# risingwavelabs/risingwave

Measured on NVIDIA H100. Metric: Nexmark q7/q8-shaped streaming HashJoin input rows/s, higher is better.
Workload: dtype int64

## Files before the change

risingwave_b200/csrc/join.cu:

```cuda
#include <algorithm>
#include <chrono>
#include <cstdio>
#include <cstdlib>
#include <memory>
#include <mutex>
#include <thread>

#include <cub/device/device_radix_sort.cuh>
#include <cub/device/device_scan.cuh>

#include "common.cuh"

namespace rw {

#define J_EMPTY 0x8000000000000000ull
#define J_NIL 0x7fffffffu
#define J_DEAD 0x80000000u
#define J_MAX_OUT (2 * RW_MAX_COLS)
#define J_HDR 16
#define W_EMPTY 0x7fffffffull
#define W_COUNT_ONE (1ull << 33)
#define W_IL_LIVE (1ull << 31)
#define W_IL_DEAD (2ull << 31)
#define W_IL_MASK (3ull << 31)
// ... 1268 lines not shown
      DevBuf b;
      const cudaError_t e = b.reserve((size_t)U_SEG_RECS * 48);
      std::lock_guard<std::mutex> g(mu);
      if (e == cudaSuccess) { spare = std::move(b); spare_ready = true; } else { cudaGetLastError(); }
      worker_running = false;
    });
  }
  int ensure(uint64_t rows, cudaStream_t st) {
    if (!table.p) {
      RW_CUDA(table.reserve(U_MAX_SEGS * sizeof(void*)));
      RW_CUDA(cudaMemsetAsync(table.p, 0, U_MAX_SEGS * sizeof(void*), st));
    }
    while (cap() < rows) {
      if (segs.size() >= U_MAX_SEGS) return fail(RW_ERR_OOM, "join side exceeds 2^31 log rows");
      DevBuf sg;
      if (worker.joinable()) worker.join();
      {
        std::lock_guard<std::mutex> g(mu);
        if (spare_ready) { sg = std::move(spare); spare_ready = false; prefetched++; }
      }
      if (!sg.p) {
        cudaError_t e = sg.reserve((size_t)U_SEG_RECS * 48);
        if (e != cudaSuccess) { cudaGetLastError(); return fail(RW_ERR_OOM, std::string("join log segment: ") + cudaGetErrorString(e)); }
        stalls++;
      }
      void* ptr = sg.p;
      RW_CUDA(cudaMemcpyAsync(table.as<uint8_t>() + segs.size() * sizeof(void*), &ptr, sizeof(void*), cudaMemcpyHostToDevice, st));
      segs.push_back(std::move(sg));
    }
    return RW_OK;
  }
};

struct JoinSideHost {
  int n_cols = 0;
  std::vector<int> types;
  SegLog log;
  GrowBuf recs;
  DevBuf slots;
  DevBuf pools;
  int stride = 0, bstride = 0;
  uint64_t row_cap = 0;
  uint64_t n_rows = 0;
  uint64_t slot_cap = 0;
  uint64_t keys_upper = 0;
};

struct JoinPending {
  int S = 0, set = 0, grid = 0;
  DevChunk ch;
  cudaStream_t st = nullptr;
  int64_t out_base = 0;
  bool plain = true, counted = false, sync_done = false;
  uint32_t pool_chunk = 0;
  uint64_t seq_base = 0, ids_before = 0, keys_before = 0;
  unsigned long long tag = 0;
  int64_t rows = 0;
  unsigned long long nullm = 0;
};

struct rwgpu_join {
  JoinPlanDev plan;
  DevBuf plan_dev, status;
  PinnedBuf status_host;
  JoinSideHost side[2];
  cudaStream_t stream = nullptr, s_h2d = nullptr, s_d2h = nullptr;
  cudaEvent_t ev_h2d[8] = {nullptr}, ev_main[8] = {nullptr};
  std::vector<int> out_types;
  int chunk_size = 1024;
  bool fast_inner = false;
  bool w8_ok[2] = {false, false};
  W8Plan w8[2];
  bool uni = false;
  int uni_is = 1;
  DevBuf uni_buckets, uni_counters;
  uint64_t uni_cap = 0, uni_keys = 0, uni_keys_exact = 0;
  uint64_t uni_dead[2] = {0, 0};
  uint64_t compactions = 0;
  DevBuf uni_wk_entry, uni_wk_mask;
  int64_t uni_wk_cap = 0;
  JoinPending pending[2];
  int n_pending = 0;
  cudaEvent_t pend_ev[2] = {nullptr, nullptr};
  cudaStream_t last_st = nullptr;
  cudaEvent_t order_ev = nullptr;
  bool wm_pending[2] = {false, false};
  int wm_key_pos[2] = {0, 0};
  int64_t wm_value[2] = {0, 0};
  uint64_t wm_cleanings = 0;
  uint64_t launches = 0;
  uint64_t seq = 0;
  unsigned long long status_tag = 0;
  unsigned long long call_null_mask = 0;
  bool out_rows_cumulative = false;
  KernelProf prof;
  DevBuf sk, sk_alt, packed, offs, mslot, gtable, cub_tmp;
  int64_t scratch_rows = 0;
  uint64_t gcap = 0;
  size_t cub_bytes = 0;
  struct OutSet {
    DevBuf out_ops, out_vis, out_col[J_MAX_OUT], out_valid[J_MAX_OUT], out_bits[J_MAX_OUT], out_visbits;
    int64_t out_cap = 0;
    unsigned long long valid_dirty = 0;
  } oset[2];
  int cur = 0;
  OutSet& os() { return oset[cur]; }
// ... 283 lines not shown
static int join_order(rwgpu_join* h, cudaStream_t st) {
  if (h->last_st && h->last_st != st) {
    if (!h->order_ev) RW_CUDA(cudaEventCreateWithFlags(&h->order_ev, cudaEventDisableTiming));
    RW_CUDA(cudaEventRecord(h->order_ev, h->last_st));
    RW_CUDA(cudaStreamWaitEvent(st, h->order_ev, 0));
  }
  h->last_st = st;
  return RW_OK;
}

static int uni_tail_grid(int64_t n) {
  static int max_blocks = 0;
  if (!max_blocks) {
    int dev = 0, sms = 0, per_sm = 0;
    cudaGetDevice(&dev);
    cudaDeviceGetAttribute(&sms, cudaDevAttrMultiProcessorCount, dev);
    int a = 0, b = 0;
    cudaOccupancyMaxActiveBlocksPerMultiprocessor(&a, uni_tail_kernel<false>, 256, 0);
    cudaOccupancyMaxActiveBlocksPerMultiprocessor(&b, uni_tail_kernel<true>, 256, 0);
    per_sm = std::max(1, std::min(std::min(a, b), 3));
    max_blocks = std::max(1, sms * per_sm);
  }
  return (int)std::max<int64_t>(1, std::min<int64_t>((n + 255) / 256, max_blocks));
}

static int uni_launch_main(rwgpu_join* h, const JoinPending& pd, bool probe_only, unsigned long long tag) {
  UniDev t = uni_dev(h);
  const JoinPlanDev* pdev = h->plan_dev.as<JoinPlanDev>();
  JoinStatus* ds = h->status.as<JoinStatus>();
  int S = pd.S;
  const bool is_row = S == h->uni_is;
  JoinOutDev od = out_dev(h);
  UniWork wk;
  wk.entry = h->uni_wk_entry.as<UniDefer>();
  wk.mask = h->uni_wk_mask.as<uint8_t>();
  W8Plan w = h->w8[S];
  h->prof.begin(pd.st);
  if (pd.plain) {
    PlainChunk pc;
    pc.ops = pd.ch.ops;
    for (int c = 0; c < 4; c++) pc.c[c] = c < w.n_u ? (const unsigned long long*)pd.ch.cols[c].data : nullptr;
    pc.key = (const unsigned long long*)pd.ch.cols[w.key_col].data;
    pc.n = pd.ch.n;
    pc.n_dev = pd.ch.n_dev;
    UniOwn own;
    own.log = t.log[S];
    own.log_cap = t.log_cap[S];
    own.pools = t.pools[S];
    own.log_next = t.log_next[S];
    PlainOut po;
    po.ops = od.ops;
    po.vis = od.vis;
    for (int c = 0; c < 4; c++) {
      po.ucol[c] = (c < w.n_u && w.u_out[c] >= 0) ? (unsigned long long*)od.col[w.u_out[c]] : nullptr;
      po.mcol[c] = (c < w.n_m && w.m_out[c] >= 0) ? (unsigned long long*)od.col[w.m_out[c]] : nullptr;
    }
    po.capacity = od.capacity;
    auto hot = probe_only ? (is_row ? uni_hot_kernel<true, true> : uni_hot_kernel<true, false>)
                          : (is_row ? uni_hot_kernel<false, true> : uni_hot_kernel<false, false>);
    hot<<<pd.grid, JF_BLOCK, 0, pd.st>>>(pc, t.buckets, t.cap, own, po, wk, ds, pd.seq_base, pd.out_base, pd.pool_chunk);
  } else {
    if (probe_only) uni_slow_kernel<true><<<jgrid(pd.ch.n, 256), 256, 0, pd.st>>>(pdev, w, S, pd.ch, t, od, ds, pd.seq_base, pd.out_base);
    else uni_slow_kernel<false><<<jgrid(pd.ch.n, 256), 256, 0, pd.st>>>(pdev, w, S, pd.ch, t, od, ds, pd.seq_base, pd.out_base);
  }
  h->prof.end(pd.st);
  RW_CUDA(cudaGetLastError());
  DevChunk chv = pd.ch;
  uint64_t seq_base = pd.seq_base;
  int64_t out_base = pd.out_base;
  JoinStatus* slot = (JoinStatus*)(h->status_host.as<uint8_t>() + 512 * pd.set);
  int reset = 3;
  unsigned int* done = (unsigned int*)(h->uni_counters.as<unsigned long long>() + 6);
  const int tg = uni_tail_grid(pd.ch.n);
  if (probe_only) uni_tail_kernel<true><<<tg, 256, 0, pd.st>>>(pdev, w, S, chv, t, od, wk, ds, seq_base, out_base, slot, tag, reset, done);
  else uni_tail_kernel<false><<<tg, 256, 0, pd.st>>>(pdev, w, S, chv, t, od, wk, ds, seq_base, out_base, slot, tag, reset, done);
  RW_CUDA(cudaGetLastError());
  h->launches += 2;
  return RW_OK;
}

static int join_plain_chunk(DevChunk* ch, bool device_count, cudaStream_t st, bool* plain) {
  *plain = ch->vis_bits == nullptr;
  for (int c = 0; c < ch->n_cols && *plain; c++)
    *plain = !ch->cols[c].valid_bits && !ch->cols[c].valid_bytes && (((uintptr_t)ch->cols[c].data & 7) == 0);
  if (!ch->n_dev || (device_count && *plain)) return RW_OK;
  int64_t nh = 0;
  RW_CUDA(cudaMemcpyAsync(&nh, ch->n_dev, sizeof(nh), cudaMemcpyDeviceToHost, st));
  RW_CUDA(cudaStreamSynchronize(st));
  if (nh < 0 || nh > ch->n) return fail(RW_ERR_INVALID, "device row count out of range");
  ch->n = nh;
  ch->n_dev = nullptr;
  return RW_OK;
}

static double uni_now_ms() { return std::chrono::duration<double, std::milli>(std::chrono::steady_clock::now().time_since_epoch()).count(); }
static const bool uni_trace = getenv("RWGPU_TRACE") != nullptr;

static int uni_enqueue(rwgpu_join* h, int S, const DevChunk& ch_in, cudaStream_t st, int64_t out_base, JoinPending* pd) {
  const double tr0 = uni_trace ? uni_now_ms() : 0.0;
  DevChunk ch = ch_in;
  bool plain_cols;
  int rc = join_plain_chunk(&ch, true, st, &plain_cols);
  if (rc != RW_OK) return rc;
  const bool counted = ch.n_dev != nullptr;
  const int64_t n = ch.n;
  JoinSideHost& own = h->side[S];
  const int grid = (int)std::max<int64_t>(1, std::min<int64_t>((n + 63) / 64, U_MAX_GRID));
  uint32_t pool_chunk = 32;
  while (pool_chunk < 256 && (int64_t)pool_chunk * grid * 8 < 4 * n) pool_chunk <<= 1;
  const uint64_t id_slack = (uint64_t)grid * 8 * pool_chunk;
  rc = join_grow_store(h, S, own.n_rows + (uint64_t)n + id_slack);
  if (rc != RW_OK) return rc;
  rc = uni_grow_table(h, h->uni_keys + (uint64_t)n);
  if (rc != RW_OK) return rc;
  rc = join_ensure_out(h, out_base + n + std::max<int64_t>(n / 2, 4096), st, out_base);
  if (rc != RW_OK) return rc;
  if (plain_cols && n > h->uni_wk_cap) {
    RW_CUDA(cudaDeviceSynchronize());
    const int64_t cap = n + n / 4 + 64;
    RW_CUDA(h->uni_wk_entry.reserve((size_t)cap * sizeof(UniDefer)));
    RW_CUDA(h->uni_wk_mask.reserve((size_t)(cap + 7) / 8 + 16));
    h->uni_wk_cap = cap;
  }
  rc = join_order(h, st);
  if (rc != RW_OK) return rc;
  const double tr1 = uni_trace ? uni_now_ms() : 0.0;
  pd->S = S;
  pd->ch = ch;
  pd->st = st;
  pd->out_base = out_base;
  pd->set = h->cur;
  pd->plain = plain_cols;
  pd->counted = counted;
  pd->grid = grid;
  pd->pool_chunk = pool_chunk;
  pd->seq_base = h->seq;
  pd->tag = ++h->status_tag;
  pd->ids_before = own.n_rows;
  pd->keys_before = h->uni_keys;
  h->seq += (uint64_t)n;
  own.n_rows += (uint64_t)n + id_slack;
  h->uni_keys += (uint64_t)n;
  rc = uni_launch_main(h, *pd, false, pd->tag);
  if (rc != RW_OK) return rc;
  if (!h->pend_ev[pd->set]) RW_CUDA(cudaEventCreateWithFlags(&h->pend_ev[pd->set], cudaEventDisableTiming));
  RW_CUDA(cudaEventRecord(h->pend_ev[pd->set], st));
  if (uni_trace)
    fprintf(stderr, "  [uni_enqueue S=%d n=%lld set=%d] grow/ensure %.3f ms, launch %.3f ms (log segs %zu/%zu, cap %llu keys<=%llu)\n", S, (long long)n,
            pd->set, tr1 - tr0, uni_now_ms() - tr1, h->side[0].log.segs.size(), h->side[1].log.segs.size(), (unsigned long long)h->uni_cap,
            (unsigned long long)h->uni_keys);
  return RW_OK;
}

static int uni_finish(rwgpu_join* h, const JoinPending& pd, int64_t* out_rows, unsigned long long* null_mask) {
  cudaStream_t st = pd.st;
  JoinStatus* ds = h->status.as<JoinStatus>();
  JoinStatus* slot = (JoinStatus*)(h->status_host.as<uint8_t>() + 512 * pd.set);
  JoinStatus hs;
  const double tr0 = uni_trace ? uni_now_ms() : 0.0;
  RW_CUDA(cudaEventSynchronize(h->pend_ev[pd.set]));
  const double tr1 = uni_trace ? uni_now_ms() : 0.0;
  int rc;
  if (*(volatile unsigned long long*)(slot + 1) != pd.tag) return fail(RW_ERR_CUDA, "join status block was not published");
  memcpy(&hs, slot, sizeof(JoinStatus));
  unsigned int err = hs.err;
  const unsigned long long first_null = hs.null_mask;
  const bool first_match = hs.pad != 0;
  const unsigned long long first_del = hs.n_del;
  const bool redone = (hs.err & JERR_OUT_CAPACITY) != 0;
  if (redone) {
    const int64_t extras = (int64_t)hs.out_rows, n = pd.ch.n;
    RW_CUDA(cudaMemsetAsync(&ds->err, 0, 4, st));
    rc = join_ensure_out(h, pd.out_base + n + extras + (int64_t)pd.grid * 8 * U_XCHUNK, st, pd.out_base);
    if (rc != RW_OK) return rc;
    const unsigned long long tag2 = ++h->status_tag;
    rc = uni_launch_main(h, pd, true, tag2);
    if (rc != RW_OK) return rc;
    RW_CUDA(cudaStreamSynchronize(st));
    if (*(volatile unsigned long long*)(slot + 1) != tag2) return fail(RW_ERR_CUDA, "join status block was not published");
    memcpy(&hs, slot, sizeof(JoinStatus));
    err = (err & ~JERR_OUT_CAPACITY) | hs.err;
    hs.null_mask |= first_null & ~(1ull << 63);
    hs.pad = hs.pad || first_match;
    hs.n_del = first_del;
  }
  for (int s = 0; s < 2; s++) h->uni_dead[s] = hs.n_dead[s];
  {
    JoinSideHost& own = h->side[pd.S];
    const uint64_t n = (uint64_t)pd.ch.n, slack = (uint64_t)pd.grid * 8 * pd.pool_chunk;
    const uint64_t rows_now = hs.log_next[pd.S] + (own.n_rows - (pd.ids_before + n + slack));
    const uint64_t keys_now = hs.n_keys[0] + (h->uni_keys - (pd.keys_before + n));
    for (int i = 0; i < h->n_pending; i++) {
      h->pending[i].ids_before += rows_now - own.n_rows;
      h->pending[i].keys_before += keys_now - h->uni_keys;
    }
    own.n_rows = rows_now;
    h->uni_keys = keys_now;
    h->uni_keys_exact = hs.n_keys[0];
  }
  hs.err = err;
  rc = join_check_err(h, hs, st);
  if (rc != RW_OK) return rc;
  const int64_t n_eff = pd.counted ? (int64_t)hs.n_in : pd.ch.n;
  *out_rows = (hs.pad != 0 || hs.out_rows) ? n_eff + (int64_t)hs.out_rows : 0;
  h->call_null_mask |= hs.null_mask;
  *null_mask = h->call_null_mask;
  h->os().valid_dirty |= hs.null_mask & ((1ull << 63) - 1);
  if (hs.n_del) h->call_had_deletes = true;
  if (uni_trace)
    fprintf(stderr, "  [uni_finish S=%d set=%d] wait %.3f ms, rest %.3f ms (redo %d, extras %llu, n_del %llu, out %lld)\n", pd.S, pd.set, tr1 - tr0,
            uni_now_ms() - tr1, (int)redone, (unsigned long long)hs.out_rows,
            (unsigned long long)hs.n_del, (long long)*out_rows);
  return RW_OK;
}

static int join_push_dev_uni(rwgpu_join* h, int S, const DevChunk& ch_in, cudaStream_t st, int64_t out_base, int64_t* out_rows,
                             unsigned long long* null_mask) {
  if (h->n_pending) return fail(RW_ERR_INVALID, "collect the outstanding asynchronous pushes first");
  JoinPending pd;
  int rc = uni_enqueue(h, S, ch_in, st, out_base, &pd);
  if (rc != RW_OK) return rc;
  return uni_finish(h, pd, out_rows, null_mask);
}

static int join_push_dev(rwgpu_join* h, int S, const DevChunk& ch_in, cudaStream_t st, int64_t out_base, int64_t* out_rows,
                         unsigned long long* null_mask) {
  *out_rows = 0;
  DevChunk ch = ch_in;
  if (ch.n <= 0) return RW_OK;
  if (ch.n >= (1ll << 31)) return fail(RW_ERR_INVALID, "chunk too large");
  if (h->uni) return join_push_dev_uni(h, S, ch_in, st, out_base, out_rows, null_mask);
  bool plain_cols;
  int rc = join_plain_chunk(&ch, false, st, &plain_cols);
  if (rc != RW_OK) return rc;
  if (ch.n == 0) return RW_OK;
  const int64_t n = ch.n;
  JoinSideHost& own = h->side[S];
  static const bool trace = getenv("RWGPU_TRACE") != nullptr;
  auto now = []() { return std::chrono::duration<double, std::milli>(std::chrono::steady_clock::now().time_since_epoch()).count(); };
  const double tt0 = now();
  const uint64_t cap0 = own.slot_cap, rcap0 = own.row_cap;
  rc = join_grow_store(h, S, own.n_rows + (uint64_t)n);
  if (rc != RW_OK) return rc;
  rc = join_grow_slots(h, S, own.keys_upper + (uint64_t)n);
  if (rc != RW_OK) return rc;
  if (trace)
    fprintf(stderr, "  [push_dev S=%d n=%lld] grow %.3f ms (slot_cap %llu->%llu, row_cap %llu->%llu, n_rows %llu keys %llu)\n", S, (long long)n,
            now() - tt0, (unsigned long long)cap0, (unsigned long long)own.slot_cap, (unsigned long long)rcap0,
            (unsigned long long)own.row_cap, (unsigned long long)own.n_rows, (unsigned long long)own.keys_upper);
  JoinStatus* ds = h->status.as<JoinStatus>();
  const JoinPlanDev* pd = h->plan_dev.as<JoinPlanDev>();
  const uint64_t seq_base = h->seq;
  h->seq += (uint64_t)n;
  JoinStatus hs;
  if (h->fast_inner) {
    const bool use_w8 = h->w8_ok[S] && plain_cols;
    if (use_w8) {
      rc = join_ensure_out(h, out_base + n + std::max<int64_t>(n / 2, 4096), st, out_base);
      if (rc != RW_OK) return rc;
      const int grid = jgrid(n, JF_BLOCK);
      auto launch = [&](bool probe_only, uint32_t store_base) {
        if (probe_only)
          join_inner_w8p_kernel<true><<<grid, JF_BLOCK, 0, st>>>(pd, h->w8[S], S, ch, side_dev(h, S), side_dev(h, 1 - S), out_dev(h), ds,
                                                                  store_base, seq_base, out_base);
        else
          join_inner_w8p_kernel<false><<<grid, JF_BLOCK, 0, st>>>(pd, h->w8[S], S, ch, side_dev(h, S), side_dev(h, 1 - S), out_dev(h), ds,
                                                                   store_base, seq_base, out_base);
      };
      h->prof.begin(st);
      launch(false, (uint32_t)own.n_rows);
      h->prof.end(st);
      const unsigned long long tag = ++h->status_tag;
      join_inner_delete_kernel<<<jgrid(n, 256), 256, 0, st>>>(pd, S, ch, side_dev(h, S), ds, seq_base, h->status_host.as<JoinStatus>(), tag, 3);
      RW_CUDA(cudaGetLastError());
      h->launches += 2;
      rc = join_read_status(h, st, &hs, 3, tag);
      if (rc != RW_OK) return rc;
      const uint64_t stored = hs.n_store, keys = hs.n_keys[S];
      if (hs.n_del) h->call_had_deletes = true;
      unsigned int err = hs.err;
      if (hs.err & JERR_OUT_CAPACITY) {
        const int64_t extras = (int64_t)hs.out_rows;
        RW_CUDA(cudaMemsetAsync(&ds->out_rows, 0, 8, st));
        RW_CUDA(cudaMemsetAsync(&ds->err, 0, 4, st));
// ... 401 lines not shown
  if (n == 0) { RW_CUDA(cudaMemsetAsync(vo.offs.p, 0, 4, st)); return RW_OK; }
  varlen_lens_kernel<<<jgrid(n, 256), 256, 0, st>>>(handles, vis, valid, n, vo.lens.as<uint32_t>());
  size_t tb = vo.tmp_bytes;
  cub::DeviceScan::ExclusiveSum(vo.tmp.p, tb, vo.lens.as<uint32_t>(), vo.offs.as<uint32_t>(), (int)n, st);
  varlen_total_kernel<<<1, 1, 0, st>>>(vo.lens.as<uint32_t>(), vo.offs.as<uint32_t>(), n);
  RW_CUDA(cudaGetLastError());
  uint32_t total = 0;
  RW_CUDA(cudaMemcpyAsync(&total, vo.offs.as<uint32_t>() + n, 4, cudaMemcpyDeviceToHost, st));
  RW_CUDA(cudaStreamSynchronize(st));
  vo.total = total;
  RW_CUDA(vo.bytes.reserve((size_t)total + 16));
  if (total) {
    varlen_gather_kernel<<<jgrid(n, 256), 256, 0, st>>>(handles, vo.offs.as<uint32_t>(), n, h->var_heap[0].as<uint8_t>(), h->var_heap[1].as<uint8_t>(),
                                                         vo.bytes.as<uint8_t>());
    RW_CUDA(cudaGetLastError());
  }
  h->launches += 4;
  return RW_OK;
}

static int var_intern_device_chunk(rwgpu_join* h, int side, const rw_chunk* c, DevChunk* ch, cudaStream_t st) {
  if (h->var_in[side].empty()) return RW_OK;
  if (ch->n_dev) return fail(RW_ERR_UNSUPPORTED, "a device-resident row count with varlen columns");
  const int64_t n = c->n_rows;
  for (int k : h->var_in[side]) {
    if (n && !c->columns[k].offsets) return fail(RW_ERR_INVALID, "varlen column without offsets");
    uint32_t o0 = 0, o1 = 0;
    if (n) {
      RW_CUDA(cudaMemcpyAsync(&o0, c->columns[k].offsets, 4, cudaMemcpyDeviceToHost, st));
      RW_CUDA(cudaMemcpyAsync(&o1, c->columns[k].offsets + n, 4, cudaMemcpyDeviceToHost, st));
      RW_CUDA(cudaStreamSynchronize(st));
    }
    int rc = var_ensure_heap(h, side, (uint64_t)(o1 - o0) + 8ull * (uint64_t)n);
    if (rc != RW_OK) return rc;
    h->var_upper[side] += (uint64_t)(o1 - o0) + 8ull * (uint64_t)n;
    RW_CUDA(h->var_handles[k].reserve((size_t)std::max<int64_t>(n, 1) * 8));
    rc = var_intern(h, side, (const uint8_t*)c->columns[k].data, c->columns[k].offsets, c->ops, c->visibility, c->columns[k].validity, n,
                    h->var_handles[k].as<uint64_t>(), st);
    if (rc != RW_OK) return rc;
    ch->cols[k].data = h->var_handles[k].p;
  }
  return var_check_err(h, st);
}

static int join_post_process(rwgpu_join* h, int64_t n, unsigned long long* nullm, cudaStream_t st) {
  if (!h->call_had_deletes || n < 2) return RW_OK;
  bool hid = false;
  int rc = join_eliminate_noop(h, n, !h->call_vis_stale, st, &hid);
  if (rc != RW_OK) return rc;
  if (hid) *nullm |= 1ull << 63;
  return RW_OK;
}

static int join_fill_view(rwgpu_join* h, int64_t n, unsigned long long nullm, rw_chunk* view, cudaStream_t st) {
  std::vector<rw_column>& cols = h->dev_view_cols[h->cur];
  cols.resize(h->out_types.size());
  for (size_t k = 0; k < h->out_types.size(); k++) {
    rw_column& col = cols[k];
    col.type = h->out_types[k];
    col.reserved = 0;
    col.data = h->os().out_col[k].p;
    col.validity = nullptr;
    col.offsets = nullptr;
    if (type_is_varlen(h->out_types[k])) {
      rwgpu_join::VarOut& vo = h->vout[h->cur][k];
      int rc = var_materialize(h, vo, h->os().out_col[k].as<uint64_t>(), (nullm >> 63) ? h->os().out_vis.as<uint8_t>() : nullptr,
                               ((nullm >> k) & 1) ? h->os().out_valid[k].as<uint8_t>() : nullptr, n, st);
      if (rc != RW_OK) return rc;
      col.data = vo.bytes.p;
      col.offsets = vo.offs.as<uint32_t>();
    }
    if (((nullm >> k) & 1) && n > 0) {
      pack_bytes_to_bits_kernel<<<jgrid((n + 63) / 64, 256), 256, 0, st>>>(h->os().out_valid[k].as<uint8_t>(), h->os().out_bits[k].as<uint64_t>(), n);
      RW_CUDA(cudaGetLastError());
      col.validity = h->os().out_bits[k].as<uint64_t>();
    }
  }
  view->n_rows = n;
  view->n_cols = (int32_t)h->out_types.size();
  view->reserved = 0;
  view->ops = h->os().out_ops.as<uint8_t>();
  view->visibility = nullptr;
  if ((nullm >> 63) && n > 0) {
    pack_bytes_to_bits_kernel<<<jgrid((n + 63) / 64, 256), 256, 0, st>>>(h->os().out_vis.as<uint8_t>(), h->os().out_visbits.as<uint64_t>(), n);
    RW_CUDA(cudaGetLastError());
    view->visibility = h->os().out_visbits.as<uint64_t>();
  }
  view->columns = cols.data();
  return RW_OK;
}

int32_t rwgpu_join_push_device_counted(rwgpu_join* h, int32_t side, const rw_chunk* c, const int64_t* n_rows_dev, rw_chunk* view,
                                       void* cuda_stream) {
  if (!h || !c || !view) return fail(RW_ERR_INVALID, "null");
  if (side != 0 && side != 1) return fail(RW_ERR_INVALID, "side");
  if (c->n_cols != h->side[side].n_cols) return fail(RW_ERR_INVALID, "chunk schema mismatch");
  if (h->n_pending) return fail(RW_ERR_INVALID, "collect the outstanding asynchronous pushes first");
  DevChunk ch;
  int rc = devchunk_from_abi(c, &ch);
  if (rc != RW_OK) return rc;
  ch.n_dev = n_rows_dev;
  cudaStream_t st = cuda_stream ? (cudaStream_t)cuda_stream : h->stream;
  int64_t n = 0;
  unsigned long long nullm = 0;
  rc = join_begin_call(h, st);
  if (rc != RW_OK) return rc;
  rc = var_intern_device_chunk(h, side, c, &ch, st);
  if (rc != RW_OK) return rc;
  rc = join_push_dev(h, side, ch, st, 0, &n, &nullm);
  if (rc != RW_OK) return rc;
  rc = join_post_process(h, n, &nullm, st);
  if (rc != RW_OK) return rc;
  return join_fill_view(h, n, nullm, view, st);
}

int32_t rwgpu_join_push_device_async(rwgpu_join* h, int32_t side, const rw_chunk* c, const int64_t* n_rows_dev, void* cuda_stream) {
  if (!h || !c) return fail(RW_ERR_INVALID, "null");
  if (side != 0 && side != 1) return fail(RW_ERR_INVALID, "side");
  if (c->n_cols != h->side[side].n_cols) return fail(RW_ERR_INVALID, "chunk schema mismatch");
  if (h->n_pending >= 2) return fail(RW_ERR_INVALID, "two pushes are already outstanding: collect one first");
  if (h->n_pending && h->pending[0].S != side)
    return fail(RW_ERR_INVALID, "pushes of different sides cannot be outstanding together: collect first");
  DevChunk ch;
  int rc = devchunk_from_abi(c, &ch);
  if (rc != RW_OK) return rc;
  ch.n_dev = n_rows_dev;
  cudaStream_t st = cuda_stream ? (cudaStream_t)cuda_stream : h->stream;
  h->cur = h->n_pending ? 1 - h->pending[h->n_pending - 1].set : h->cur;
  rc = join_begin_call(h, st);
  if (rc != RW_OK) return rc;
  JoinPending pd;
  rc = var_intern_device_chunk(h, side, c, &ch, st);
  if (rc != RW_OK) return rc;
  if (h->uni && ch.n > 0 && ch.n < (1ll << 31) && h->var_in[side].empty()) {
    rc = uni_enqueue(h, side, ch, st, 0, &pd);
    if (rc != RW_OK) return rc;
  } else {
    pd.S = side;
    pd.set = h->cur;
    pd.st = st;
    pd.sync_done = true;
    rc = join_push_dev(h, side, ch, st, 0, &pd.rows, &pd.nullm);
    if (rc != RW_OK) return rc;
    rc = join_post_process(h, pd.rows, &pd.nullm, st);
    if (rc != RW_OK) return rc;
  }
  h->pending[h->n_pending++] = pd;
  return RW_OK;
}

int32_t rwgpu_join_collect(rwgpu_join* h, rw_chunk* view, void* cuda_stream) {
  if (!h || !view) return fail(RW_ERR_INVALID, "null");
  if (h->n_pending == 0) return fail(RW_ERR_INVALID, "no push outstanding");
  const JoinPending pd = h->pending[0];
  if (h->hpend[pd.set].active) return fail(RW_ERR_INVALID, "the oldest outstanding push was launched with a host chunk: use rwgpu_join_collect_out");
  h->pending[0] = h->pending[1];
  h->n_pending--;
  h->cur = pd.set;
  int64_t n = pd.rows;
  unsigned long long nullm = pd.nullm;
  if (!pd.sync_done) {
    h->call_null_mask = 0;
    h->call_had_deletes = false;
    int rc = uni_finish(h, pd, &n, &nullm);
    if (rc != RW_OK) return rc;
    const double tp0 = uni_trace ? uni_now_ms() : 0.0;
    rc = join_post_process(h, n, &nullm, pd.st);
    if (rc != RW_OK) return rc;
    if (uni_trace) fprintf(stderr, "  [collect] post-process (no-op elimination: %d) %.3f ms\n", (int)h->call_had_deletes, uni_now_ms() - tp0);
  }
  int rc = join_fill_view(h, n, nullm, view, cuda_stream ? (cudaStream_t)cuda_stream : pd.st);
  if (h->n_pending) h->cur = h->pending[h->n_pending - 1].set;
  return rc;
}

int32_t rwgpu_join_push(rwgpu_join* h, int32_t side, const rw_chunk* c, rwgpu_out** out) {
  if (!h || !c || !out) return fail(RW_ERR_INVALID, "null");
  if (side != 0 && side != 1) return fail(RW_ERR_INVALID, "side");
  if (c->n_cols != h->side[side].n_cols) return fail(RW_ERR_INVALID, "chunk schema mismatch");
  for (int k = 0; k < c->n_cols; k++)
    if (c->columns[k].type != h->side[side].types[k]) return fail(RW_ERR_INVALID, "chunk column type mismatch");
  if (h->n_pending) return fail(RW_ERR_INVALID, "collect the outstanding asynchronous pushes first");
  const int64_t n = c->n_rows;
  static const bool trace = getenv("RWGPU_TRACE") != nullptr;
  auto now = []() { return std::chrono::duration<double, std::milli>(std::chrono::steady_clock::now().time_since_epoch()).count(); };
  const double t0 = now();
  if (!h->s_h2d) {
    RW_CUDA(cudaStreamCreateWithFlags(&h->s_h2d, cudaStreamNonBlocking));
    RW_CUDA(cudaStreamCreateWithFlags(&h->s_d2h, cudaStreamNonBlocking));
    for (int i = 0; i < 8; i++) {
      RW_CUDA(cudaEventCreateWithFlags(&h->ev_h2d[i], cudaEventDisableTiming));
      RW_CUDA(cudaEventCreateWithFlags(&h->ev_main[i], cudaEventDisableTiming));
    }
  }
  const int J = n >= (1 << 19) ? 8 : (n >= (1 << 17) ? 4 : (n >= (1 << 16) ? 2 : 1));
  int64_t sub = (n + J - 1) / J;
  sub = (sub + 63) / 64 * 64;
  const size_t nw = (size_t)((n + 63) / 64) * 8;
  size_t off = 0;
  auto region = [&](size_t bytes) { size_t o = align_up_j(off, 256); off = o + bytes; return o; };
  const size_t o_ops = region((size_t)n), o_vis = region(nw);
  size_t o_data[RW_MAX_COLS], o_valid[RW_MAX_COLS], o_voff[RW_MAX_COLS], o_vbytes[RW_MAX_COLS];
  uint64_t var_bytes_in = 0;
  for (int k = 0; k < c->n_cols; k++) {
    o_data[k] = region((size_t)n * type_width(c->columns[k].type));
    o_valid[k] = region(nw);
    o_voff[k] = o_vbytes[k] = 0;
    if (type_is_varlen(c->columns[k].type)) {
      if (n && !c->columns[k].offsets) return fail(RW_ERR_INVALID, "varlen column without offsets");
      const size_t vb = n ? (size_t)(c->columns[k].offsets[n] - c->columns[k].offsets[0]) : 0;
      o_voff[k] = region((size_t)(n + 1) * 4);
      o_vbytes[k] = region(vb + 16);
      var_bytes_in += vb + 8ull * (uint64_t)n;
    }
  }
  if (var_bytes_in) {
    int rcv = var_ensure_heap(h, side, var_bytes_in);
    if (rcv != RW_OK) return rcv;
    h->var_upper[side] += var_bytes_in;
  }
  RW_CUDA(h->up.reserve(off + 256));
  RW_CUDA(h->up_host.reserve(off + 256));
  uint8_t* hp = h->up_host.as<uint8_t>();
  uint8_t* dp = h->up.as<uint8_t>();
// ... 201 lines not shown
  if (!h->ev_up2[set]) RW_CUDA(cudaEventCreateWithFlags(&h->ev_up2[set], cudaEventDisableTiming));
  if (!h->s_out[set]) RW_CUDA(cudaStreamCreateWithFlags(&h->s_out[set], cudaStreamNonBlocking));
  cudaStream_t sd = h->s_out[set];
  const size_t nw = (size_t)((n + 63) / 64) * 8;
  size_t off = 0;
  auto region = [&](size_t bytes) { size_t o = align_up_j(off, 256); off = o + bytes; return o; };
  const size_t o_ops = region((size_t)n), o_vis = region(nw);
  size_t o_data[RW_MAX_COLS], o_valid[RW_MAX_COLS];
  for (int k = 0; k < c->n_cols; k++) {
    o_data[k] = region((size_t)n * type_width(c->columns[k].type));
    o_valid[k] = region(nw);
  }
  if (off + 256 > h->up2[set].bytes) {
    RW_CUDA(cudaDeviceSynchronize());
    RW_CUDA(h->up2[set].reserve(off + off / 4 + 256));
    RW_CUDA(h->up2_host[set].reserve(off + off / 4 + 256));
  }
  uint8_t* hs = h->up2_host[set].as<uint8_t>();
  uint8_t* dp = h->up2[set].as<uint8_t>();
  auto is_pinned = [](const void* p) {
    cudaPointerAttributes a;
    if (cudaPointerGetAttributes(&a, p) != cudaSuccess) { cudaGetLastError(); return false; }
    return a.type == cudaMemoryTypeHost;
  };
  auto h2d = [&](size_t dst_off, const void* src, size_t bytes, bool pinned) {
    if (!bytes) return;
    if (pinned || bytes >= (1u << 20)) cudaMemcpyAsync(dp + dst_off, src, bytes, cudaMemcpyHostToDevice, h->s_h2d);
    else { memcpy(hs + dst_off, src, bytes); cudaMemcpyAsync(dp + dst_off, hs + dst_off, bytes, cudaMemcpyHostToDevice, h->s_h2d); }
  };
  h2d(o_ops, c->ops, (size_t)n, is_pinned(c->ops));
  if (c->visibility) h2d(o_vis, c->visibility, nw, false);
  for (int k = 0; k < c->n_cols; k++) {
    h2d(o_data[k], c->columns[k].data, (size_t)n * type_width(c->columns[k].type), is_pinned(c->columns[k].data));
    if (c->columns[k].validity) h2d(o_valid[k], c->columns[k].validity, nw, false);
  }
  RW_CUDA(cudaEventRecord(h->ev_up2[set], h->s_h2d));
  RW_CUDA(cudaGetLastError());
  DevChunk ch;
  memset(&ch, 0, sizeof(ch));
  ch.n = n;
  ch.n_cols = c->n_cols;
  ch.ops = dp + o_ops;
  ch.vis_bits = c->visibility ? (const uint64_t*)(dp + o_vis) : nullptr;
  for (int k = 0; k < c->n_cols; k++) {
    ch.cols[k].type = c->columns[k].type;
    ch.cols[k].width = type_width(c->columns[k].type);
    ch.cols[k].data = dp + o_data[k];
    ch.cols[k].valid_bits = c->columns[k].validity ? (const uint64_t*)(dp + o_valid[k]) : nullptr;
  }
  h->cur = set;
  int rc = join_begin_call(h, h->stream);
  if (rc != RW_OK) { hp.active = false; return rc; }
  RW_CUDA(cudaStreamWaitEvent(h->stream, h->ev_up2[set], 0));
  rc = uni_enqueue(h, side, ch, h->stream, 0, &pd);
  if (rc != RW_OK) { hp.active = false; return rc; }
  auto o = new rwgpu_out();
  o->chunk_size = h->chunk_size;
  hp.host_cap = std::max<int64_t>(2 * n, 1024);
  if (!o->layout(hp.host_cap, h->out_types, ~0ull >> 1, true, h->pool)) { delete o; hp.active = false; return fail(RW_ERR_OOM, "pinned output block"); }
  hp.out = o;
  static const bool no_alias = getenv("RWGPU_NO_ALIAS") != nullptr;
  hp.alias_ok = !no_alias && h->w8_ok[side] && !c->visibility;
  for (int k = 0; k < c->n_cols && hp.alias_ok; k++) hp.alias_ok = c->columns[k].validity == nullptr;
  hp.alias_src.assign(h->out_types.size(), -1);
  if (hp.alias_ok)
    for (int k = 0; k < c->n_cols; k++)
      if (h->w8[side].u_out[k] >= 0) hp.alias_src[(size_t)h->w8[side].u_out[k]] = k;
  RW_CUDA(cudaStreamWaitEvent(sd, h->pend_ev[set], 0));
  cudaMemcpyAsync(o->ops, h->os().out_ops.p, (size_t)n, cudaMemcpyDeviceToHost, sd);
  for (size_t k = 0; k < h->out_types.size(); k++) {
    if (hp.alias_src[k] >= 0) continue;
    const size_t w = type_width(h->out_types[k]);
    cudaMemcpyAsync(o->data[k], h->os().out_col[k].p, (size_t)n * w, cudaMemcpyDeviceToHost, sd);
  }
  RW_CUDA(cudaGetLastError());
  h->pending[h->n_pending++] = pd;
  return RW_OK;
}

int32_t rwgpu_join_collect_out(rwgpu_join* h, rwgpu_out** out) {
  if (!h || !out) return fail(RW_ERR_INVALID, "null");
  if (h->n_pending == 0) return fail(RW_ERR_INVALID, "no push outstanding");
  const JoinPending pd = h->pending[0];
  rwgpu_join::HostPending& hp = h->hpend[pd.set];
  if (!hp.active) return fail(RW_ERR_INVALID, "the oldest outstanding push was launched with a device chunk: use rwgpu_join_collect");
  h->pending[0] = h->pending[1];
  h->n_pending--;
  hp.active = false;
  if (hp.sync_done) {
    *out = hp.out;
    hp.out = nullptr;
    return RW_OK;
  }
  std::unique_ptr<rwgpu_out> guard(hp.out);
  hp.out = nullptr;
  rwgpu_out* o = guard.get();
  cudaStream_t sd = h->s_out[pd.set];
  h->cur = pd.set;
  h->call_null_mask = 0;
  h->call_had_deletes = false;
  int64_t total = 0;
  unsigned long long nullm = 0;
  const uint8_t* ops_before = h->os().out_ops.as<uint8_t>();
  auto bail = [&](int rc) { cudaStreamSynchronize(sd); if (h->n_pending) h->cur = h->pending[h->n_pending - 1].set; return rc; };
  int rc = uni_finish(h, pd, &total, &nullm);
  if (rc != RW_OK) return bail(rc);
  rc = join_post_process(h, total, &nullm, pd.st);
// ... 224 lines not shown
```

risingwave_b200/device.py:

```python
from __future__ import annotations

import ctypes as C
from typing import List, Optional, Sequence

import torch

from . import abi

TORCH_DTYPE = {abi.T_BOOL: torch.uint8, abi.T_INT16: torch.int16, abi.T_INT32: torch.int32, abi.T_INT64: torch.int64,
               abi.T_FLOAT32: torch.float32, abi.T_FLOAT64: torch.float64, abi.T_DATE: torch.int32,
               abi.T_TIME: torch.int64, abi.T_TIMESTAMP: torch.int64, abi.T_TIMESTAMPTZ: torch.int64,
               abi.T_SERIAL: torch.int64}


class DeviceChunk:

    def __init__(self, ops: torch.Tensor, cols: Sequence[torch.Tensor], types: Sequence[int],
                 validity: Optional[Sequence[Optional[torch.Tensor]]] = None, visibility: Optional[torch.Tensor] = None):
        assert ops.dtype == torch.uint8 and ops.is_cuda and ops.is_contiguous()
        self.ops, self.cols, self.types = ops, list(cols), list(types)
        self.validity = list(validity) if validity is not None else [None] * len(cols)
        self.visibility = visibility
        for c, t in zip(self.cols, self.types):
            assert c.is_cuda and c.is_contiguous() and c.dtype == TORCH_DTYPE[t] and c.numel() == ops.numel()

    def n_rows(self) -> int:
        return self.ops.numel()

    def to_abi(self):
        cached = getattr(self, "_abi", None)
        if cached is not None:
            return cached
        cols = (abi.RwColumn * max(1, len(self.cols)))()
        for k, (c, t) in enumerate(zip(self.cols, self.types)):
            cols[k].type = t
            cols[k].data = c.data_ptr() if c.numel() else None
            cols[k].validity = self.validity[k].data_ptr() if self.validity[k] is not None else None
        ch = abi.RwChunk()
        ch.n_rows = self.ops.numel()
        ch.n_cols = len(self.cols)
        ch.ops = self.ops.data_ptr() if self.ops.numel() else None
        ch.visibility = self.visibility.data_ptr() if self.visibility is not None else None
        ch.columns = cols
        self._abi = (ch, cols)
        return ch, cols


class DeviceView:

    def __init__(self, view: abi.RwChunk, stream: Optional[torch.cuda.Stream] = None):
        self._stream = stream
        self._synced = False
        self.n_rows = int(view.n_rows)
        self.n_cols = int(view.n_cols)
        self.ops_ptr = view.ops
        self.vis_ptr = view.visibility
        self.col_ptrs = [view.columns[k].data for k in range(self.n_cols)]
        self.col_types = [int(view.columns[k].type) for k in range(self.n_cols)]
        self.valid_ptrs = [view.columns[k].validity for k in range(self.n_cols)]

    def _wait(self):
        if not self._synced:
            if self._stream is not None:
                self._stream.synchronize()
            else:
                torch.cuda.synchronize()
            self._synced = True

    def column(self, k: int) -> torch.Tensor:
        self._wait()
        t = self.col_types[k]
        out = torch.empty(self.n_rows, dtype=TORCH_DTYPE[t], device="cuda")
        if self.n_rows:
            _d2d(out.data_ptr(), self.col_ptrs[k], self.n_rows * abi.TYPE_WIDTH[t])
        return out

    def ops(self) -> torch.Tensor:
        self._wait()
        out = torch.empty(self.n_rows, dtype=torch.uint8, device="cuda")
        if self.n_rows:
            _d2d(out.data_ptr(), self.ops_ptr, self.n_rows)
        return out

    def visible(self) -> Optional[torch.Tensor]:
        if not self.vis_ptr or not self.n_rows:
            return None
        self._wait()
        nw = (self.n_rows + 63) // 64
        words = torch.empty(nw, dtype=torch.int64, device="cuda")
        _d2d(words.data_ptr(), self.vis_ptr, nw * 8)
        bits = (words.unsqueeze(1) >> torch.arange(64, device="cuda", dtype=torch.int64).unsqueeze(0)) & 1
        return bits.reshape(-1)[:self.n_rows].to(torch.bool)

    def checksum(self, weights: Sequence[int]) -> tuple:
        if not self.n_rows:
            return 0, 0
        acc = torch.zeros(self.n_rows, dtype=torch.int64, device="cuda")
        for k, w in enumerate(weights):
            acc += self.column(k).to(torch.int64) * int(w)
        ops = self.ops()
        sign = torch.where((ops == abi.OP_INSERT) | (ops == abi.OP_UPDATE_INSERT), 1, -1).to(torch.int64)
        acc *= sign
        vis = self.visible()
        if vis is not None:
            acc = acc[vis]
# ... 63 lines not shown
        lib.rwgpu_join_collect.argtypes = [C.c_void_p, C.POINTER(abi.RwChunk), C.c_void_p]
        lib.rwgpu_shuffle_exchange_p2p_device.restype = C.c_int32
        lib.rwgpu_shuffle_exchange_p2p_device.argtypes = [C.POINTER(abi.RwChunk), C.POINTER(C.c_int32), C.c_int32, C.c_int32, C.c_void_p,
                                                          C.c_int32, C.c_int32, C.POINTER(C.c_void_p), C.POINTER(C.c_void_p), C.c_uint64,
                                                          C.c_int64, C.c_void_p, C.c_void_p, C.POINTER(C.c_void_p), C.c_void_p,
                                                          C.c_void_p, C.c_void_p, C.c_void_p]
        lib.rwgpu_filter_device.restype = C.c_int32
        lib.rwgpu_filter_device.argtypes = [C.POINTER(abi.RwChunk), C.POINTER(abi.RwFilterTerm), C.c_int32, C.c_int32, C.c_void_p,
                                            C.c_void_p, C.c_void_p, C.c_void_p]
        lib.rwgpu_last_error.restype = C.c_char_p
        lib._dev_sigs = True
    return lib


def _check(rc):
    if rc != abi.RW_OK:
        raise abi.RwError(rc, (_lib().rwgpu_last_error() or b"").decode())


def _stream_ptr(stream: Optional[torch.cuda.Stream]):
    return C.c_void_p(stream.cuda_stream) if stream is not None else None


def agg_push_device(executor, chunk: DeviceChunk, stream: Optional[torch.cuda.Stream] = None):
    ch, keep = chunk.to_abi()
    _check(_lib().rwgpu_agg_push_device(executor._h, C.byref(ch), _stream_ptr(stream)))


def agg_flush_device(executor, epoch: int, stream: Optional[torch.cuda.Stream] = None) -> DeviceView:
    view = abi.RwChunk()
    _check(_lib().rwgpu_agg_flush_device(executor._h, epoch, C.byref(view), _stream_ptr(stream)))
    return DeviceView(view, stream)


def agg_flush_device_async(executor, epoch: int, stream: Optional[torch.cuda.Stream] = None):
    _check(_lib().rwgpu_agg_flush_device_async(executor._h, epoch, _stream_ptr(stream)))


def agg_flush_collect(executor, stream: Optional[torch.cuda.Stream] = None) -> DeviceView:
    view = abi.RwChunk()
    _check(_lib().rwgpu_agg_flush_collect(executor._h, C.byref(view), _stream_ptr(stream)))
    return DeviceView(view, stream)


def join_push_device(executor, side: int, chunk: DeviceChunk, stream: Optional[torch.cuda.Stream] = None,
                     n_rows_dev: Optional[int] = None) -> DeviceView:
    ch, keep = chunk.to_abi()
    view = abi.RwChunk()
    if n_rows_dev is None:
        _check(_lib().rwgpu_join_push_device(executor._h, side, C.byref(ch), C.byref(view), _stream_ptr(stream)))
    else:
        _check(_lib().rwgpu_join_push_device_counted(executor._h, side, C.byref(ch), C.c_void_p(n_rows_dev), C.byref(view),
                                                     _stream_ptr(stream)))
    return DeviceView(view, stream)


def join_push_device_async(executor, side: int, chunk: DeviceChunk, stream: Optional[torch.cuda.Stream] = None,
                           n_rows_dev: Optional[int] = None):
    ch, keep = chunk.to_abi()
    _check(_lib().rwgpu_join_push_device_async(executor._h, side, C.byref(ch), C.c_void_p(n_rows_dev) if n_rows_dev else None,
                                               _stream_ptr(stream)))


def join_collect(executor, stream: Optional[torch.cuda.Stream] = None) -> DeviceView:
    view = abi.RwChunk()
    _check(_lib().rwgpu_join_collect(executor._h, C.byref(view), _stream_ptr(stream)))
    return DeviceView(view, stream)


def profile(executor, kind: str, enable: bool):
    ms, n = C.c_double(), C.c_uint64()
    fn = _lib().rwgpu_agg_profile if kind == "agg" else _lib().rwgpu_join_profile
    _check(fn(executor._h, int(enable), C.byref(ms), C.byref(n)))
    return ms.value, n.value


def launches(executor, kind: str) -> int:
    a, b, c = C.c_uint64(), C.c_uint64(), C.c_uint64()
    fn = _lib().rwgpu_agg_stats if kind == "agg" else _lib().rwgpu_join_stats
    _check(fn(executor._h, C.byref(a), C.byref(b), C.byref(c)))
    return c.value


def shuffle_partition(chunk: DeviceChunk, key_indices: Sequence[int], vnode_to_dest: torch.Tensor, n_dest: int,
                      vnode_count: int = 256, stream: Optional[torch.cuda.Stream] = None):
    n = chunk.n_rows()
    out_ops = torch.empty(n, dtype=torch.uint8, device="cuda")
    out_cols = [torch.empty_like(c) for c in chunk.cols]
    counts = torch.zeros(n_dest, dtype=torch.int64, device="cuda")
    offsets = torch.zeros(n_dest, dtype=torch.int64, device="cuda")
    ch, keep = chunk.to_abi()
    keys = (C.c_int32 * len(key_indices))(*key_indices)
    colp = (C.c_void_p * len(out_cols))(*[c.data_ptr() for c in out_cols])
    _check(_lib().rwgpu_shuffle_partition_device(C.byref(ch), keys, len(key_indices), vnode_count,
                                                 C.c_void_p(vnode_to_dest.data_ptr()), n_dest, C.c_void_p(out_ops.data_ptr()),
                                                 colp, None, C.c_void_p(counts.data_ptr()), C.c_void_p(offsets.data_ptr()),
                                                 _stream_ptr(stream)))
    return out_ops, out_cols, counts, offsets


def p2p_region_bytes(types: Sequence[int], cap_rows: int) -> int:
    t = (C.c_int32 * len(types))(*types)
    out = C.c_int64()
    _check(_lib().rwgpu_shuffle_p2p_region_bytes(t, len(types), cap_rows, C.byref(out)))
    return out.value


def shuffle_partition_p2p(chunk: DeviceChunk, key_indices: Sequence[int], vnode_to_dest: torch.Tensor, n_dest: int, my_rank: int,
                          peer_ptrs: Sequence[int], cap_rows: int, counts: torch.Tensor, overflow: torch.Tensor,
                          vnode_count: int = 256, stream: Optional[torch.cuda.Stream] = None):
    ch, keep = chunk.to_abi()
    keys = (C.c_int32 * len(key_indices))(*key_indices)
    peers = (C.c_void_p * n_dest)(*peer_ptrs)
    _check(_lib().rwgpu_shuffle_partition_p2p_device(C.byref(ch), keys, len(key_indices), vnode_count,
                                                     C.c_void_p(vnode_to_dest.data_ptr()), n_dest, my_rank, peers, cap_rows,
                                                     C.c_void_p(counts.data_ptr()), C.c_void_p(overflow.data_ptr()), _stream_ptr(stream)))


def shuffle_unpack(recv_ptr: int, n_src: int, types: Sequence[int], cap_rows: int, out_ops: torch.Tensor,
                   out_cols: Sequence[torch.Tensor], total: torch.Tensor, stream: Optional[torch.cuda.Stream] = None):
# ... 97 lines not shown
```

Baseline: 5.012 billion.

## Alias unique-side output columns to input chunk buffers instead of copying

When a plain, uncounted chunk is pushed at output offset zero with no variable-length interning, the hot kernel no longer writes the pass-through (unique-side) columns into the output buffer. If the result has no extra rows and no deletes, the returned view points those columns directly at the input chunk's device memory. Otherwise a device-to-device memcpy fills them after the fact. The Python wrapper keeps the input chunk alive alongside the view so the aliased memory stays valid. This cuts output write bandwidth in the common case, at the cost of lifetime coupling and an extra copy on the fallback path.

```diff
diff --git a/risingwave_b200/csrc/join.cu b/risingwave_b200/csrc/join.cu
--- a/risingwave_b200/csrc/join.cu
+++ b/risingwave_b200/csrc/join.cu
@@ -1344,6 +1344,7 @@
   cudaStream_t st = nullptr;
   int64_t out_base = 0;
   bool plain = true, counted = false, sync_done = false;
+  bool alias_u = false;
   uint32_t pool_chunk = 0;
   uint64_t seq_base = 0, ids_before = 0, keys_before = 0;
   unsigned long long tag = 0;
@@ -1733,7 +1734,7 @@
     po.ops = od.ops;
     po.vis = od.vis;
     for (int c = 0; c < 4; c++) {
-      po.ucol[c] = (c < w.n_u && w.u_out[c] >= 0) ? (unsigned long long*)od.col[w.u_out[c]] : nullptr;
+      po.ucol[c] = (!pd.alias_u && c < w.n_u && w.u_out[c] >= 0) ? (unsigned long long*)od.col[w.u_out[c]] : nullptr;
       po.mcol[c] = (c < w.n_m && w.m_out[c] >= 0) ? (unsigned long long*)od.col[w.m_out[c]] : nullptr;
     }
     po.capacity = od.capacity;
@@ -1777,7 +1778,7 @@
 static double uni_now_ms() { return std::chrono::duration<double, std::milli>(std::chrono::steady_clock::now().time_since_epoch()).count(); }
 static const bool uni_trace = getenv("RWGPU_TRACE") != nullptr;
 
-static int uni_enqueue(rwgpu_join* h, int S, const DevChunk& ch_in, cudaStream_t st, int64_t out_base, JoinPending* pd) {
+static int uni_enqueue(rwgpu_join* h, int S, const DevChunk& ch_in, cudaStream_t st, int64_t out_base, bool alias_ok, JoinPending* pd) {
   const double tr0 = uni_trace ? uni_now_ms() : 0.0;
   DevChunk ch = ch_in;
   bool plain_cols;
@@ -1813,6 +1814,7 @@
   pd->set = h->cur;
   pd->plain = plain_cols;
   pd->counted = counted;
+  pd->alias_u = alias_ok && plain_cols && !counted && out_base == 0 && h->var_in[S].empty();
   pd->grid = grid;
   pd->pool_chunk = pool_chunk;
   pd->seq_base = h->seq;
@@ -1833,7 +1835,7 @@
   return RW_OK;
 }
 
-static int uni_finish(rwgpu_join* h, const JoinPending& pd, int64_t* out_rows, unsigned long long* null_mask) {
+static int uni_finish(rwgpu_join* h, const JoinPending& pd, int64_t* out_rows, unsigned long long* null_mask, bool* aliased = nullptr) {
   cudaStream_t st = pd.st;
   JoinStatus* ds = h->status.as<JoinStatus>();
   JoinStatus* slot = (JoinStatus*)(h->status_host.as<uint8_t>() + 512 * pd.set);
@@ -1888,6 +1890,14 @@
   *null_mask = h->call_null_mask;
   h->os().valid_dirty |= hs.null_mask & ((1ull << 63) - 1);
   if (hs.n_del) h->call_had_deletes = true;
+  const bool alias = pd.alias_u && !redone && hs.out_rows == 0 && !h->call_had_deletes;
+  if (pd.alias_u && !alias && *out_rows > 0) {
+    const W8Plan& w = h->w8[pd.S];
+    for (int c = 0; c < w.n_u; c++)
+      if (w.u_out[c] >= 0)
+        RW_CUDA(cudaMemcpyAsync(h->os().out_col[w.u_out[c]].p, pd.ch.cols[c].data, (size_t)pd.ch.n * 8, cudaMemcpyDeviceToDevice, st));
+  }
+  if (aliased) *aliased = alias;
   if (uni_trace)
     fprintf(stderr, "  [uni_finish S=%d set=%d] wait %.3f ms, rest %.3f ms (redo %d, extras %llu, n_del %llu, out %lld)\n", pd.S, pd.set, tr1 - tr0,
             uni_now_ms() - tr1, (int)redone, (unsigned long long)hs.out_rows,
@@ -1896,21 +1906,22 @@
 }
 
 static int join_push_dev_uni(rwgpu_join* h, int S, const DevChunk& ch_in, cudaStream_t st, int64_t out_base, int64_t* out_rows,
-                             unsigned long long* null_mask) {
+                             unsigned long long* null_mask, bool* aliased) {
   if (h->n_pending) return fail(RW_ERR_INVALID, "collect the outstanding asynchronous pushes first");
   JoinPending pd;
-  int rc = uni_enqueue(h, S, ch_in, st, out_base, &pd);
+  int rc = uni_enqueue(h, S, ch_in, st, out_base, aliased != nullptr, &pd);
   if (rc != RW_OK) return rc;
-  return uni_finish(h, pd, out_rows, null_mask);
+  return uni_finish(h, pd, out_rows, null_mask, aliased);
 }
 
 static int join_push_dev(rwgpu_join* h, int S, const DevChunk& ch_in, cudaStream_t st, int64_t out_base, int64_t* out_rows,
-                         unsigned long long* null_mask) {
+                         unsigned long long* null_mask, bool* aliased = nullptr) {
   *out_rows = 0;
+  if (aliased) *aliased = false;
   DevChunk ch = ch_in;
   if (ch.n <= 0) return RW_OK;
   if (ch.n >= (1ll << 31)) return fail(RW_ERR_INVALID, "chunk too large");
-  if (h->uni) return join_push_dev_uni(h, S, ch_in, st, out_base, out_rows, null_mask);
+  if (h->uni) return join_push_dev_uni(h, S, ch_in, st, out_base, out_rows, null_mask, aliased);
   bool plain_cols;
   int rc = join_plain_chunk(&ch, false, st, &plain_cols);
   if (rc != RW_OK) return rc;
@@ -2418,7 +2429,8 @@
   return RW_OK;
 }
 
-static int join_fill_view(rwgpu_join* h, int64_t n, unsigned long long nullm, rw_chunk* view, cudaStream_t st) {
+static int join_fill_view(rwgpu_join* h, int64_t n, unsigned long long nullm, rw_chunk* view, cudaStream_t st, const DevChunk* alias_in = nullptr,
+                          int S = 0) {
   std::vector<rw_column>& cols = h->dev_view_cols[h->cur];
   cols.resize(h->out_types.size());
   for (size_t k = 0; k < h->out_types.size(); k++) {
@@ -2442,6 +2454,9 @@
       col.validity = h->os().out_bits[k].as<uint64_t>();
     }
   }
+  if (alias_in)
+    for (int c = 0; c < h->w8[S].n_u; c++)
+      if (h->w8[S].u_out[c] >= 0) cols[(size_t)h->w8[S].u_out[c]].data = alias_in->cols[c].data;
   view->n_rows = n;
   view->n_cols = (int32_t)h->out_types.size();
   view->reserved = 0;
@@ -2473,11 +2488,12 @@
   if (rc != RW_OK) return rc;
   rc = var_intern_device_chunk(h, side, c, &ch, st);
   if (rc != RW_OK) return rc;
-  rc = join_push_dev(h, side, ch, st, 0, &n, &nullm);
+  bool aliased = false;
+  rc = join_push_dev(h, side, ch, st, 0, &n, &nullm, &aliased);
   if (rc != RW_OK) return rc;
   rc = join_post_process(h, n, &nullm, st);
   if (rc != RW_OK) return rc;
-  return join_fill_view(h, n, nullm, view, st);
+  return join_fill_view(h, n, nullm, view, st, aliased ? &ch : nullptr, side);
 }
 
 int32_t rwgpu_join_push_device_async(rwgpu_join* h, int32_t side, const rw_chunk* c, const int64_t* n_rows_dev, void* cuda_stream) {
@@ -2499,7 +2515,7 @@
   rc = var_intern_device_chunk(h, side, c, &ch, st);
   if (rc != RW_OK) return rc;
   if (h->uni && ch.n > 0 && ch.n < (1ll << 31) && h->var_in[side].empty()) {
-    rc = uni_enqueue(h, side, ch, st, 0, &pd);
+    rc = uni_enqueue(h, side, ch, st, 0, true, &pd);
     if (rc != RW_OK) return rc;
   } else {
     pd.S = side;
@@ -2525,17 +2541,18 @@
   h->cur = pd.set;
   int64_t n = pd.rows;
   unsigned long long nullm = pd.nullm;
+  bool aliased = false;
   if (!pd.sync_done) {
     h->call_null_mask = 0;
     h->call_had_deletes = false;
-    int rc = uni_finish(h, pd, &n, &nullm);
+    int rc = uni_finish(h, pd, &n, &nullm, &aliased);
     if (rc != RW_OK) return rc;
     const double tp0 = uni_trace ? uni_now_ms() : 0.0;
     rc = join_post_process(h, n, &nullm, pd.st);
     if (rc != RW_OK) return rc;
     if (uni_trace) fprintf(stderr, "  [collect] post-process (no-op elimination: %d) %.3f ms\n", (int)h->call_had_deletes, uni_now_ms() - tp0);
   }
-  int rc = join_fill_view(h, n, nullm, view, cuda_stream ? (cudaStream_t)cuda_stream : pd.st);
+  int rc = join_fill_view(h, n, nullm, view, cuda_stream ? (cudaStream_t)cuda_stream : pd.st, aliased ? &pd.ch : nullptr, pd.S);
   if (h->n_pending) h->cur = h->pending[h->n_pending - 1].set;
   return rc;
 }
@@ -2843,7 +2860,7 @@
   int rc = join_begin_call(h, h->stream);
   if (rc != RW_OK) { hp.active = false; return rc; }
   RW_CUDA(cudaStreamWaitEvent(h->stream, h->ev_up2[set], 0));
-  rc = uni_enqueue(h, side, ch, h->stream, 0, &pd);
+  rc = uni_enqueue(h, side, ch, h->stream, 0, false, &pd);
   if (rc != RW_OK) { hp.active = false; return rc; }
   auto o = new rwgpu_out();
   o->chunk_size = h->chunk_size;
diff --git a/risingwave_b200/device.py b/risingwave_b200/device.py
--- a/risingwave_b200/device.py
+++ b/risingwave_b200/device.py
@@ -1,5 +1,6 @@
 from __future__ import annotations
 
+import collections
 import ctypes as C
 from typing import List, Optional, Sequence
 
@@ -48,9 +49,10 @@
 
 class DeviceView:
 
-    def __init__(self, view: abi.RwChunk, stream: Optional[torch.cuda.Stream] = None):
+    def __init__(self, view: abi.RwChunk, stream: Optional[torch.cuda.Stream] = None, chunk: Optional[DeviceChunk] = None):
         self._stream = stream
         self._synced = False
+        self._chunk = chunk
         self.n_rows = int(view.n_rows)
         self.n_cols = int(view.n_cols)
         self.ops_ptr = view.ops
@@ -220,7 +222,7 @@
     else:
         _check(_lib().rwgpu_join_push_device_counted(executor._h, side, C.byref(ch), C.c_void_p(n_rows_dev), C.byref(view),
                                                      _stream_ptr(stream)))
-    return DeviceView(view, stream)
+    return DeviceView(view, stream, chunk)
 
 
 def join_push_device_async(executor, side: int, chunk: DeviceChunk, stream: Optional[torch.cuda.Stream] = None,
@@ -228,12 +230,17 @@
     ch, keep = chunk.to_abi()
     _check(_lib().rwgpu_join_push_device_async(executor._h, side, C.byref(ch), C.c_void_p(n_rows_dev) if n_rows_dev else None,
                                                _stream_ptr(stream)))
+    if not hasattr(executor, "_pushed_chunks"):
+        executor._pushed_chunks = collections.deque()
+    executor._pushed_chunks.append(chunk)
 
 
 def join_collect(executor, stream: Optional[torch.cuda.Stream] = None) -> DeviceView:
     view = abi.RwChunk()
+    pushed = getattr(executor, "_pushed_chunks", None)
+    chunk = pushed.popleft() if pushed else None
     _check(_lib().rwgpu_join_collect(executor._h, C.byref(view), _stream_ptr(stream)))
-    return DeviceView(view, stream)
+    return DeviceView(view, stream, chunk)
 
 
 def profile(executor, kind: str, enable: bool):
```

Measured after the change: 5.384 billion (median of 6 runs). 1.07x the previous value.
